# SokhengDin/DNN-MPPI-MPC

Hardware: NVIDIA B200
Metric: mppi_sample_steps_per_sec (higher is better)
Workload: dtype f32

## Files before the change

dnn-mppi-mpc_b200/csrc/mppi_api.cu:

```cuda
#include <cuda_runtime.h>
#include <dlfcn.h>
#include <nccl.h>

#include <algorithm>
#include <cmath>
#include <cstdio>
#include <cstdlib>
#include <cstring>
#include <string>
#include <vector>

#include "mppi_device.cuh"
#include "mppi_launch.h"
#include "mppi_mlp.h"

namespace {

struct NcclApi {
    void *lib = nullptr;
    ncclResult_t (*GetUniqueId)(ncclUniqueId *) = nullptr;
    ncclResult_t (*CommInitRank)(ncclComm_t *, int, ncclUniqueId, int) = nullptr;
    ncclResult_t (*AllGather)(const void *, void *, size_t, ncclDataType_t, ncclComm_t, cudaStream_t) = nullptr;
    ncclResult_t (*CommDestroy)(ncclComm_t) = nullptr;
    const char *(*GetErrorString)(ncclResult_t) = nullptr;
// ... 281 lines not shown
            h->grid_x_tpar = gt;
            gx = std::max(gx, gt);
        }
    }

    CKC(gmalloc(h, &h->d_U, sizeof(float) * R * T * 2));
    CKC(cudaMemset(h->d_U, 0, sizeof(float) * R * T * 2));
    CKC(gmalloc(h, &h->d_M, sizeof(float) * T * T));
    CKC(gmalloc(h, &h->d_S, sizeof(float) * (size_t)R * K));
    CKC(gmalloc(h, &h->d_NC, sizeof(int) * (size_t)K));
    const int gmax = (gx + MPPI_MERGE_GROUP_CTAS - 1) / MPPI_MERGE_GROUP_CTAS;
    CKC(gmalloc(h, &h->d_part, sizeof(float) * (size_t)R * (gx + gmax) * MPPI_NF(T)));
    CKC(gmalloc(h, &h->d_out, sizeof(float) * (size_t)R * MPPI_OUT_STRIDE));
    CKC(cudaMemset(h->d_out, 0, sizeof(float) * (size_t)R * MPPI_OUT_STRIDE));
    CKC(gmalloc(h, &h->d_idx, sizeof(int) * R));
    CKC(cudaMemset(h->d_idx, 0, sizeof(int) * R));
    CKC(gmalloc(h, &h->d_ticket, sizeof(unsigned) * (size_t)R * (1 + gmax)));
    CKC(cudaMemset(h->d_ticket, 0, sizeof(unsigned) * (size_t)R * (1 + gmax)));
    CKC(cudaHostAlloc(&h->h_out, sizeof(float) * MPPI_OUT_STRIDE, cudaHostAllocMapped));
    std::memset(h->h_out, 0, sizeof(float) * MPPI_OUT_STRIDE);
    CKC(cudaHostGetDevicePointer(&h->h_out_dev, h->h_out, 0));
    CKC(gmalloc(h, &h->d_first, sizeof(unsigned long long)));
    CKC(cudaHostAlloc(&h->h_first, sizeof(unsigned long long), cudaHostAllocDefault));
    h->idx_mirror = 0; h->idx_mirror_ok = true;
    for (auto &e : h->ev) CKC(cudaEventCreate(&e));
    std::vector<float> M;
    build_filter(T, c.filter_kind, M);
    CKC(cudaMemcpy(h->d_M, M.data(), sizeof(float) * T * T, cudaMemcpyHostToDevice));

    TickArgs &a = h->args;
    std::memset(&a, 0, sizeof(a));
    a.K = K; a.T = T; a.window = c.window; a.yaw_wrap = c.yaw_wrap; a.clamp_nominal = c.clamp_nominal;
    a.k_offset = c.k_offset;
    {
        const double thr = (1.0 - c.param_exploration) * (double)c.K_global;
        long long n = (long long)std::ceil(thr);
        n = std::max(0LL, std::min((long long)c.K_global, n));
        a.n_exploit = (int)n;
    }
    a.dt = (float)c.dt; a.dt_over_L = (float)(c.dt / c.wheel_base);
    a.umax0 = (float)c.u_max[0]; a.umax1 = (float)c.u_max[1];
    for (int i = 0; i < 4; ++i) { a.sw[i] = (float)c.stage_w[i]; a.tw[i] = (float)c.term_w[i]; }
    const double gamma = c.param_lambda * (1.0 - c.param_alpha);
    a.use_gamma = gamma != 0.0;
    a.gq[0] = (float)(gamma * c.sigma[3] / det); a.gq[1] = (float)(-gamma * c.sigma[1] / det);
    a.gq[2] = (float)(-gamma * c.sigma[2] / det); a.gq[3] = (float)(gamma * c.sigma[0] / det);
    const double l00 = std::sqrt(c.sigma[0]), l10 = c.sigma[2] / l00;
    a.chol[0] = (float)l00; a.chol[1] = (float)l10; a.chol[2] = (float)std::sqrt(c.sigma[3] - l10 * l10);
    a.inv_temp = (float)(1.0 / c.temperature);
    for (int i = 0; i < 4; ++i) a.goal[i] = (float)c.goal[i];
    a.ctrl_w[0] = (float)c.ctrl_w[0]; a.ctrl_w[1] = (float)c.ctrl_w[1];
    a.soft_w = (float)c.soft_obs_weight; a.soft_sd = (float)c.soft_obs_safety;
    refresh_obstacle_args(h, nullptr, 0);
    a.U = h->d_U; a.idx = h->d_idx; a.M = h->d_M; a.part = h->d_part; a.ticket = h->d_ticket;
    a.part2 = h->d_part + (size_t)R * gx * MPPI_NF(T); a.ticket2 = h->d_ticket + R; a.merge_gmax = gmax;
    a.out = h->d_out; a.out_host = h->h_out_dev;
    if (c.model == MPPI_MODEL_DIFFDRIVE_MLP) {
        h->mlp = mlp_create(K, T);
        if (!h->mlp) { mppi_destroy(h); return MPPI_E_CUDA; }
    }
#undef CKC
    *out = h;
    return MPPI_OK;
}

int mppi_destroy(mppi_handle_t h) {
// ... 755 lines not shown
```

dnn-mppi-mpc_b200/csrc/mppi_device.cuh:

```cuda
#pragma once
#include <cuda_runtime.h>
#include <stdint.h>
#include <math_constants.h>
#include "../../include/mppi_b200.h"

#ifndef MPPI_DEBUG_CHECKS
#define MPPI_DEBUG_CHECKS 0
#endif
#if MPPI_DEBUG_CHECKS
#include <assert.h>
#define MPPI_DCHECK(c) assert(c)
#else
#define MPPI_DCHECK(c) ((void)0)
#endif
#ifndef MPPI_BLOCK
#define MPPI_BLOCK 256
#endif
#define MPPI_WARPS (MPPI_BLOCK / 32)
#ifndef MPPI_SPT
#define MPPI_SPT 1
#endif
#define MPPI_CHUNK (MPPI_BLOCK * MPPI_SPT)
#ifndef MPPI_MIN_BLOCKS
#define MPPI_MIN_BLOCKS (MPPI_BLOCK >= 512 ? 1 : 768 / MPPI_BLOCK)
// ... 17 lines not shown
#define MPPI_XCHG_TOTAL (MPPI_XCHG_BARRIER + MPPI_MAX_PEERS)

enum : int {
    F_WRITE_S = 1,
    F_UPDATE = 2,
    F_FROM_S = 4,
    F_HOST_IDX = 8,
    F_TRIPLE_OUT = 16,
    F_KEEP_IDX = 32,
    F_IDX_ONLY = 64,
    F_P2P = 128,
    F_COST_SUM = 0x10000
};

struct TickArgs {
    int K, T, window, n_path, n_obs, yaw_wrap, use_gamma, clamp_nominal;
    int k_offset, n_exploit;
    float dt, dt_over_L, umax0, umax1;
    float sw[4], tw[4];
    float gq[4];
    float chol[3];
    float inv_temp;
    float obs_x[MPPI_MAX_OBSTACLES], obs_y[MPPI_MAX_OBSTACLES];
    float obs_r2[MPPI_MAX_OBSTACLES];
    float obs_far2[MPPI_MAX_OBSTACLES];
    float fp_hl, fp_hw;
    float goal[4];
    float ctrl_w[2];
    float soft_w, soft_sd;
    float obs_vx[MPPI_MAX_OBSTACLES], obs_vy[MPPI_MAX_OBSTACLES];
    float x0[4];
    uint32_t seed_lo, seed_hi, tick;
    int idx_host, flags;
    const float4 *path;
    const int *path_len;
    int path_stride;
    const float *x0_dev;
    float *U;
    int *idx;
    const float *M;
    const float *eps;
    float *S;
    int *NC;
    float *S_user;
    float *part;
    unsigned *ticket;
    float *part2;
    unsigned *ticket2;
    int merge_gmax;
    float *out;
    float *out_host;
    float *u0_out;
    float *triple_out;
    float *plant_state;
    float *plant_log;
    int plant_mode, plant_tick, plant_n;
    unsigned *loop_state;
    unsigned *loop_ticket;
    unsigned long long *peer_buf[MPPI_MAX_PEERS];
    int p2p_rank, p2p_world;
    unsigned p2p_seq;
    unsigned p2p_timeout_ms;
    unsigned long long *trace;
};

__device__ __forceinline__ void philox4x32_10(uint32_t &c0, uint32_t &c1, uint32_t &c2, uint32_t &c3,
// ... 324 lines not shown
#endif
    auto far = [&](int ch) {
        const float4 cb = sm.cb[ch];
        const float ex = x - cb.x, ey = y - cb.y, R = sbm + cb.z;
        return fmaf(ey, ey, ex * ex) > R * R * 1.0002f;
    };
#if MPPI_WP_CHUNK_ILP
    for (; c + 1 < nch; c += 2) {
        if (far(c) && far(c + 1)) continue;
        float m0, k0, m1, k1;
        chunk_argmin<16>(nwx4 + 4 * c, nwy4 + 4 * c, x, y, m0, k0);
        chunk_argmin<16>(nwx4 + 4 * c + 4, nwy4 + 4 * c + 4, x, y, m1, k1);
        const bool second = m1 < m0;
        const float m = second ? m1 : m0;
        const int j = second ? 16 * c + 16 + __float2int_rn(k1) : 16 * c + __float2int_rn(k0);
        if (m < bm) { bm = m; bj = j; sbm = sqrtf(m); }
    }
#endif
    for (; c < nch; ++c) {
        if (far(c)) continue;
        float m, key;
        chunk_argmin<16>(nwx4 + 4 * c, nwy4 + 4 * c, x, y, m, key);
        if (m < bm) { bm = m; bj = 16 * c + __float2int_rn(key); sbm = sqrtf(m); }
    }
    return bj;
}

__device__ __forceinline__ float4 window_ref(const TickSmem &sm, int j) {
    MPPI_DCHECK(j >= 0 && j < MPPI_MAX_WINDOW);
    const float2 yv = sm.wyv[j];
    return make_float4(-sm.wx[j], -sm.wy[j], yv.x, yv.y);
}

__device__ __forceinline__ void sincos_cw(float x, float &s, float &c) {
    const float t = fmaf(x, 0.636619772f, 12582912.f);
    const int q = __float_as_int(t);
    const float k = t - 12582912.f;
    float r = fmaf(k, -1.5707963705062866f, x);
    r = fmaf(k, 4.371138828673793e-08f, r);
    r = fmaf(k, 1.7151245100058819e-15f, r);
    const float r2 = r * r;
    float sp = fmaf(r2, -1.9515295891e-4f, 8.3321608736e-3f);
    sp = fmaf(sp, r2, -1.6666654611e-1f);
    sp = fmaf(sp * r2, r, r);
    float cp = fmaf(r2, 2.443315711809948e-5f, -1.388731625493765e-3f);
    cp = fmaf(cp, r2, 4.166664568298827e-2f);
    cp = fmaf(cp, r2, -0.5f);
    cp = fmaf(cp, r2, 1.0f);
    const float ss = (q & 1) ? cp : sp, cc = (q & 1) ? sp : cp;
    s = __int_as_float(__float_as_int(ss) ^ ((q << 30) & 0x80000000));
    c = __int_as_float(__float_as_int(cc) ^ (((q + 1) << 30) & 0x80000000));
}

__device__ __forceinline__ float wrap_2pi(float yaw) {
    const float b = 6.2831855f;
    const float y2 = yaw + b;
    const float q = floorf(y2 * 0.15915494f);
    float r = fmaf(-q, b, y2);
    if (r < 0.f) r += b;
    if (r >= b) r -= b;
    return r;
}

template <int MODEL, int COLL>
__device__ __forceinline__ bool collided(const TickArgs &a, float x, float y, float cs, float sn) {
    bool hit = false;
// ... 37 lines not shown
#define MPPI_WIN_GOAL (-1)
#define MPPI_WIN_TARGET (-2)

__device__ __forceinline__ float goal_cost(const TickArgs &a, const float z[4], const float w[4]) {
    const float dx = z[0] - a.goal[0], dy = z[1] - a.goal[1];
    const float d2 = fmaf(dy, dy, dx * dx);
    const float diff = atan2f(dy, dx) - z[2];
    const float k = rintf(diff * 0.15915494309189535f);
    float r = fmaf(k, -6.2831854820251465f, diff);
    r = fmaf(k, 1.7484555314695172e-07f, r);
    return w[0] * d2 + w[1] * r * r;
}

__device__ __forceinline__ float target_soft_cost(const TickArgs &a, const float z[4], float v0, float v1, int t,
                                                  const float w[4], bool full) {
    const float ex = z[0] - a.goal[0], ey = z[1] - a.goal[1], eth = z[2] - a.goal[2];
    float c = w[0] * ex * ex + w[1] * ey * ey + w[2] * eth * eth;
    if (full) {
        c += a.ctrl_w[0] * v0 * v0 + a.ctrl_w[1] * v1 * v1;
        const float tt = (float)t * a.dt;
        float soft = 0.f;
        for (int m = 0; m < a.n_obs; ++m) {
            const float dx = z[0] - fmaf(a.obs_vx[m], tt, a.obs_x[m]), dy = z[1] - fmaf(a.obs_vy[m], tt, a.obs_y[m]);
            const float d = sqrtf(fmaf(dy, dy, dx * dx));
            if (d < a.soft_sd) soft += expf(a.soft_sd - d);
        }
        c = fmaf(a.soft_w, soft, c);
    }
    return c;
}

template <int MODEL, int WIN>
__device__ __forceinline__ float eval_state_cost(const TickArgs &a, const TickSmem &sm, const float z[4], float v0, float v1,
                                                 int t, const float w[4], float4 &ref, float &yaw_eff) {
    if constexpr (WIN == MPPI_WIN_GOAL) {
        return goal_cost(a, z, w);
    } else if constexpr (WIN == MPPI_WIN_TARGET) {
        return target_soft_cost(a, z, v0, v1, t, w, true);
    } else {
        const int j = nearest_wp<WIN>(sm, z[0], z[1]);
        ref = window_ref(sm, j);
        yaw_eff = (MODEL == MPPI_MODEL_BICYCLE && a.yaw_wrap) ? wrap_2pi(z[2]) : z[2];
        return tracking_cost<MODEL>(ref, z, yaw_eff, w);
    }
}
template <int MODEL, int WIN>
__device__ __forceinline__ float eval_terminal_cost(const TickArgs &a, const float z[4], const float4 ref, float yaw_eff) {
    if constexpr (WIN == MPPI_WIN_GOAL) return goal_cost(a, z, a.tw);
    else if constexpr (WIN == MPPI_WIN_TARGET) return target_soft_cost(a, z, 0.f, 0.f, 0, a.tw, false);
    else return tracking_cost<MODEL>(ref, z, yaw_eff, a.tw);
}

template <int MODEL>
__device__ __forceinline__ void dyn_step(const TickArgs &a, float z[4], float v0, float v1, float cs, float sn) {
    if (MODEL == MPPI_MODEL_BICYCLE) {
        const float vel = z[3];
        z[0] += vel * cs * a.dt;
        z[1] += vel * sn * a.dt;
        z[2] += vel * a.dt_over_L * tanf(v0);
        z[3] += v1 * a.dt;
    } else {
        z[0] += v0 * cs * a.dt;
        z[1] += v0 * sn * a.dt;
        z[2] += v1 * a.dt;
    }
}

template <int MODEL>
__device__ __forceinline__ void dyn_step_tan(const TickArgs &a, float z[4], float v0, float v1, float cs, float sn, float tan_v0) {
    if (MODEL == MPPI_MODEL_BICYCLE) {
        const float vel = z[3];
        z[0] += vel * cs * a.dt;
        z[1] += vel * sn * a.dt;
        z[2] += vel * a.dt_over_L * tan_v0;
        z[3] += v1 * a.dt;
    } else {
        dyn_step<MODEL>(a, z, v0, v1, cs, sn);
    }
}

__device__ __forceinline__ float clampf(float v, float lim) { return fminf(fmaxf(v, -lim), lim); }

template <int MODEL, int COLL, bool SUM, bool INJ, int WIN, int SPT>
__device__ __forceinline__ void rollout_samples(const TickArgs &a, const TickSmem &sm, const uint32_t (&kg)[SPT], const int (&klocal)[SPT],
                                                uint32_t robot, const bool (&exploit)[SPT], float2 *stash, float (&smooth)[SPT], int (&ncoll)[SPT],
                                                uint32_t tick_add = 0u) {
    const int T = a.T;
    float z[SPT][4], cs[SPT], sn[SPT], acc[SPT], v0[SPT], v1[SPT], yaw_eff[SPT];
    int nc[SPT];
    float4 ref[SPT];
    bool hit[SPT];
    const float2 *eps_k[SPT];
#pragma unroll
    for (int s = 0; s < SPT; ++s) {
        z[s][0] = sm.x0[0]; z[s][1] = sm.x0[1]; z[s][2] = sm.x0[2]; z[s][3] = sm.x0[3];
        sincos_cw(z[s][2], sn[s], cs[s]);
        acc[s] = 0.f; nc[s] = 0; v0[s] = v1[s] = 0.f; yaw_eff[s] = 0.f; hit[s] = false;
        ref[s] = make_float4(0.f, 0.f, 0.f, 0.f);
        eps_k[s] = INJ ? reinterpret_cast<const float2 *>(a.eps) + (size_t)klocal[s] * T : nullptr;
    }

    auto fetch = [&](int s, int tp, float e[4]) {
        if (INJ) {
            e[0] = e[1] = e[2] = e[3] = 0.f;
            if (tp < T) { const float2 ea = eps_k[s][tp]; e[0] = ea.x; e[1] = ea.y; }
            if (tp + 1 < T) { const float2 eb = eps_k[s][tp + 1]; e[2] = eb.x; e[3] = eb.y; }
        } else {
            philox_eps_pair(a, kg[s], (uint32_t)(tp >> 1), robot, e, tick_add);
        }
    };
    auto step = [&](int s, int t, float e0, float e1) {
        MPPI_DCHECK(t >= 0 && t < T);
        if (stash) stash[t * MPPI_CHUNK + s * MPPI_BLOCK] = make_float2(e0, e1);
        const float2 u = sm.U[t];
        v0[s] = clampf(exploit[s] ? __fadd_rn(u.x, e0) : e0, a.umax0);
        v1[s] = clampf(exploit[s] ? __fadd_rn(u.y, e1) : e1, a.umax1);
        dyn_step<MODEL>(a, z[s], v0[s], v1[s], cs[s], sn[s]);
        sincos_cw(z[s][2], sn[s], cs[s]);
        if (SUM) {
            const float c = eval_state_cost<MODEL, WIN>(a, sm, z[s], v0[s], v1[s], t, a.sw, ref[s], yaw_eff[s]);
            const float2 q = sm.Q[t];
            acc[s] += c + (q.x * v0[s] + q.y * v1[s]);
            hit[s] = collided<MODEL, COLL>(a, z[s][0], z[s][1], cs[s], sn[s]);
            nc[s] += hit[s] ? 1 : 0;
        }
    };

    float e[SPT][4];
#pragma unroll
    for (int s = 0; s < SPT; ++s) fetch(s, 0, e[s]);
    const int n_fetch_pairs = WIN >= 0 ? (T - 1) >> 1 : T >> 1;
    int tp = 0;
    for (int i = 0; i < n_fetch_pairs; ++i, tp += 2) {
        float en[SPT][4];
#pragma unroll
        for (int s = 0; s < SPT; ++s) fetch(s, tp + 2, en[s]);
#pragma unroll
        for (int s = 0; s < SPT; ++s) step(s, tp, e[s][0], e[s][1]);
#pragma unroll
        for (int s = 0; s < SPT; ++s) step(s, tp + 1, e[s][2], e[s][3]);
#pragma unroll
        for (int s = 0; s < SPT; ++s) { e[s][0] = en[s][0]; e[s][1] = en[s][1]; e[s][2] = en[s][2]; e[s][3] = en[s][3]; }
    }
#pragma unroll
    for (int s = 0; s < SPT; ++s) {
        if (WIN >= 0) {
            step(s, tp, e[s][0], e[s][1]);
            if (!(T & 1)) step(s, tp + 1, e[s][2], e[s][3]);
        } else if (T & 1) {
            step(s, T - 1, e[s][0], e[s][1]);
        }
        if (SUM) {
            acc[s] += eval_terminal_cost<MODEL, WIN>(a, z[s], ref[s], yaw_eff[s]);
            nc[s] += hit[s] ? 1 : 0;
        } else {
            const float2 q = sm.Q[T - 1];
            acc[s] = eval_state_cost<MODEL, WIN>(a, sm, z[s], v0[s], v1[s], T - 1, a.sw, ref[s], yaw_eff[s]) + (q.x * v0[s] + q.y * v1[s]);
            acc[s] += eval_terminal_cost<MODEL, WIN>(a, z[s], ref[s], yaw_eff[s]);
            nc[s] = collided<MODEL, COLL>(a, z[s][0], z[s][1], cs[s], sn[s]) ? 2 : 0;
        }
        smooth[s] = acc[s];
        ncoll[s] = nc[s];
    }
}

#define MPPI_TPAR_SLOTS 64
#ifndef MPPI_TPAR_PROBE
#define MPPI_TPAR_PROBE 0
#endif
#if MPPI_TPAR_PROBE
#include <cstdio>
#endif
struct TparSmem {
    int prog[MPPI_TPAR_SLOTS / 32];
    int next;
};
template <int MODEL, int COLL, int WIN>
__device__ __forceinline__ void rollout_tpar(const TickArgs &a, const TickSmem &sm, TparSmem &ts, const int k_begin, const int n, const uint32_t robot,
                                             float2 *stash, float4 *zbuf, float &smooth, int &ncoll, const uint32_t tick_add) {
    const int T = a.T, tid = threadIdx.x;
    const uint32_t inv_n = n > 1 ? (uint32_t)((0x100000000ull + (uint32_t)n - 1u) / (uint32_t)n) : 0u;
    auto div_n = [&](int i) { return n > 1 ? (int)__umulhi((uint32_t)i, inv_n) : i; };
    if (tid < MPPI_TPAR_SLOTS / 32) ts.prog[tid] = 0;
    if (tid == 0) ts.next = 0;
    const uint32_t kg0 = (uint32_t)(a.k_offset + k_begin);
    MPPI_DCHECK(n >= 1 && n <= MPPI_TPAR_SLOTS && MPPI_TPAR_SLOTS <= MPPI_BLOCK);
#if MPPI_TPAR_PROBE
    long long pc[5];
#define MPPI_TPAR_STAMP(i) pc[i] = clock64()
#else
#define MPPI_TPAR_STAMP(i)
#endif
    MPPI_TPAR_STAMP(0);
    {
        const int npairs = (T + 1) >> 1, items = n * npairs;
        for (int i = tid; i < items; i += MPPI_BLOCK) {
            const int p = div_n(i), slot = i - p * n;
            MPPI_DCHECK(p == i / n && 2 * p < T && slot >= 0 && slot < n);
            float e[4];
            philox_eps_pair(a, kg0 + (uint32_t)slot, (uint32_t)p, robot, e, tick_add);
            stash[(2 * p) * MPPI_TPAR_SLOTS + slot] = make_float2(e[0], e[1]);
            if (2 * p + 1 < T) stash[(2 * p + 1) * MPPI_TPAR_SLOTS + slot] = make_float2(e[2], e[3]);
            if (MODEL == MPPI_MODEL_BICYCLE) {
                const bool exploit = (int)(kg0 + (uint32_t)slot) < a.n_exploit;
                const float ua = sm.U[2 * p].x, ub = (2 * p + 1 < T) ? sm.U[2 * p + 1].x : 0.f;
                zbuf[(2 * p) * MPPI_TPAR_SLOTS + slot].x = tanf(clampf(exploit ? __fadd_rn(ua, e[0]) : e[0], a.umax0));
                if (2 * p + 1 < T) zbuf[(2 * p + 1) * MPPI_TPAR_SLOTS + slot].x = tanf(clampf(exploit ? __fadd_rn(ub, e[2]) : e[2], a.umax0));
            }
        }
        const int idle = MPPI_TPAR_SLOTS - n;
        for (int i = tid; i < idle * T; i += MPPI_BLOCK) {
            const int t = i / idle, slot = n + (i - t * idle);
// ... 28 lines not shown
                asm volatile("st.release.cta.shared.u32 [%0], %1;" ::"r"((uint32_t)__cvta_generic_to_shared(&ts.prog[warp])), "r"(done) : "memory");
            }
        }
    }
    MPPI_TPAR_STAMP(2);
    {
        const int items = n * T;
        for (;;) {
            int base = 0;
            if (lane == 0) base = atomicAdd(&ts.next, 32);
            base = __shfl_sync(0xffffffffu, base, 0);
            if (base >= items) break;
            const int i = base + lane;
            if (i < items) {
                const int t = div_n(i), slot = i - t * n;
                MPPI_DCHECK(t == i / n && t < T && slot >= 0 && slot < n && (slot >> 5) < n_dw);
                {
                    const uint32_t flag = (uint32_t)__cvta_generic_to_shared(&ts.prog[slot >> 5]);
                    int done;
                    for (;;) {
                        asm volatile("ld.acquire.cta.shared.u32 %0, [%1];" : "=r"(done) : "r"(flag) : "memory");
                        if (done > t) break;
                        __nanosleep(40);
                    }
                }
                const float4 z4 = zbuf[t * MPPI_TPAR_SLOTS + slot];
                const float z[4] = {z4.x, z4.y, z4.z, z4.w};
                const bool exploit = (int)(kg0 + (uint32_t)slot) < a.n_exploit;
                const float2 e = stash[t * MPPI_TPAR_SLOTS + slot], u = sm.U[t];
                const float v0 = clampf(exploit ? __fadd_rn(u.x, e.x) : e.x, a.umax0);
                const float v1 = clampf(exploit ? __fadd_rn(u.y, e.y) : e.y, a.umax1);
                float4 ref = make_float4(0.f, 0.f, 0.f, 0.f);
                float yaw_eff = 0.f;
                const float c = eval_state_cost<MODEL, WIN>(a, sm, z, v0, v1, t, a.sw, ref, yaw_eff);
                const float2 q = sm.Q[t];
                const float cc = c + (q.x * v0 + q.y * v1);
                bool hit = false;
                if constexpr (COLL != MPPI_COLLISION_NONE) {
                    float cs, sn;
                    sincos_cw(z[2], sn, cs);
                    hit = collided<MODEL, COLL>(a, z[0], z[1], cs, sn);
                }
                const float term = (t == T - 1) ? eval_terminal_cost<MODEL, WIN>(a, z, ref, yaw_eff) : 0.f;
                zbuf[t * MPPI_TPAR_SLOTS + slot] = make_float4(cc, term, hit ? 1.f : 0.f, 0.f);
            }
        }
    }
    __syncthreads();
    MPPI_TPAR_STAMP(3);
    smooth = CUDART_INF_F; ncoll = INT_MAX;
    if (tid < n) {
        float acc = 0.f;
        int nc = 0;
        float4 r = make_float4(0.f, 0.f, 0.f, 0.f);
        for (int t = 0; t < T; ++t) {
            r = zbuf[t * MPPI_TPAR_SLOTS + tid];
            acc += r.x;
            nc += (r.z != 0.f) ? 1 : 0;
        }
        acc += r.y;
        nc += (r.z != 0.f) ? 1 : 0;
        smooth = acc; ncoll = nc;
    }
#if MPPI_TPAR_PROBE
    MPPI_TPAR_STAMP(4);
    if (tid == 0 && (blockIdx.x == 0 || blockIdx.x == 77) && a.tick == 25u)
        printf("tpar block %d n %d: N %lld D %lld C %lld S %lld cycles\n", (int)blockIdx.x, n, pc[1] - pc[0], pc[2] - pc[1], pc[3] - pc[2], pc[4] - pc[3]);
// ... 3 lines not shown
```

dnn-mppi-mpc_b200/csrc/mppi_kernels.cu:

```cuda
#include "mppi_device.cuh"
#include "mppi_launch.h"

#include <algorithm>

namespace {

__device__ __forceinline__ float warp_sum(float v) {
#pragma unroll
    for (int o = 16; o > 0; o >>= 1) v += __shfl_xor_sync(0xffffffffu, v, o);
    return v;
}

__device__ __forceinline__ void warp_lexmin(int &n, float &s) {
    const int nmin = __reduce_min_sync(0xffffffffu, n);
    float c = (n == nmin) ? s : CUDART_INF_F;
#pragma unroll
    for (int o = 16; o > 0; o >>= 1) c = fminf(c, __shfl_xor_sync(0xffffffffu, c, o));
    n = nmin; s = c;
}

__device__ __forceinline__ float rel_weight(int n, float s, int n0, float s0, float inv_temp) {
    const float d = (float)(n - n0) * MPPI_PENALTY + (s - s0);
    return __expf(-d * inv_temp);
}

struct MergeSmem {
    float red_s[MPPI_WARPS];
    int red_n[MPPI_WARPS];
    float col[4 + 2 * MPPI_MAX_T];
    float weps[2 * MPPI_MAX_T];
    float upre[2 * MPPI_MAX_T];
};

#ifndef MPPI_MERGE_TWO_LEVEL
#define MPPI_MERGE_TWO_LEVEL 1
#endif
#define MPPI_MERGE_TWO_LEVEL_MIN 64
#define MPPI_MERGE_TILE 1000
#define MPPI_MERGE_GROUPS 4
#define MPPI_MERGE_SCRATCH (MPPI_MERGE_TILE + MPPI_MERGE_GROUPS * MPPI_NF_MAX)
static_assert(4 * MPPI_BLOCK <= MPPI_MERGE_SCRATCH || MPPI_BLOCK > 256, "merge fast path: group sums must fit the scratch");
__device__ void merge_partials(const TickArgs &a, const float *parts, int P, MergeSmem &ms, float *sc, int stride = 0) {
    const int tid = threadIdx.x, lane = tid & 31, warp = tid >> 5;
    const int NF = MPPI_NF(a.T);
    if (stride == 0) stride = NF;
    int n = INT_MAX;
    float s = CUDART_INF_F;
    int my_n = INT_MAX;
    float my_s = CUDART_INF_F;
    for (int p = tid; p < P; p += MPPI_BLOCK) {
        const int pn = __float_as_int(__ldcg(parts + (size_t)p * stride));
        const float ps = __ldcg(parts + (size_t)p * stride + 1);
        if (p == tid) { my_n = pn; my_s = ps; }
        if (pn < n || (pn == n && ps < s)) { n = pn; s = ps; }
    }
    warp_lexmin(n, s);
    if (lane == 0) { ms.red_n[warp] = n; ms.red_s[warp] = s; }
    __syncthreads();
    n = ms.red_n[0]; s = ms.red_s[0];
#pragma unroll
    for (int w = 1; w < MPPI_WARPS; ++w) {
        const int wn = ms.red_n[w]; const float ws = ms.red_s[w];
        if (wn < n || (wn == n && ws < s)) { n = wn; s = ws; }
    }
    if ((NF & 3) == 0 && (stride & 3) == 0 && MPPI_BLOCK / (NF >> 2) >= 2 && P <= MPPI_MERGE_TILE) {
        const int NQ = NF >> 2, G4 = min(MPPI_BLOCK / NQ, 16);
        const int g4 = tid / NQ, cq = tid - g4 * NQ;
        __syncthreads();
        if (tid < P) sc[tid] = rel_weight(my_n, my_s, n, s, a.inv_temp);
        for (int p = tid + MPPI_BLOCK; p < P; p += MPPI_BLOCK) {
            const float *pp = parts + (size_t)p * stride;
            sc[p] = rel_weight(__float_as_int(__ldcg(pp)), __ldcg(pp + 1), n, s, a.inv_temp);
        }
// ... 161 lines not shown
            } else {
                const float steer = clampf(u0x, a.umax0), accel = clampf(u0y, a.umax1);
                px += pv * cs * a.dt; py += pv * sn * a.dt; pyaw += pv * a.dt_over_L * tanf(steer); pv += accel * a.dt;
            }
            ps[0] = px; ps[1] = py; ps[2] = pyaw; ps[3] = pv;
            float *lg = a.plant_log + 4 * ((size_t)(pt + 1) * R + robot);
            lg[0] = px; lg[1] = py; lg[2] = pyaw; lg[3] = pv;
            float *lu = a.plant_log + 4 * (size_t)(a.plant_n + 1) * R + 2 * ((size_t)pt * R + robot);
            lu[0] = u0x; lu[1] = u0y;
        }
        if (!(a.flags & F_KEEP_IDX)) a.idx[robot] = idx_new;
    }
}

struct RunSmem {
    int n;
    float s;
    float eta, e2;
    float N[2 * MPPI_MAX_T];
    float w[MPPI_CHUNK];
    float warp_eta[MPPI_WARPS], warp_e2[MPPI_WARPS];
    float red_s[MPPI_WARPS];
    int red_n[MPPI_WARPS];
    unsigned long long key[MPPI_WARPS];
    unsigned ticket;
};

extern __shared__ __align__(16) unsigned char mppi_dyn_smem[];

template <int MODEL, int COLL, bool SUM, bool INJ, int WIN, int STASH>
__device__ __forceinline__ void tick_body(const TickArgs &a, const uint32_t tick_add) {
    __shared__ TickSmem sm;
    __shared__ RunSmem run;
    __shared__ MergeSmem ms;
    float2 *stash = reinterpret_cast<float2 *>(mppi_dyn_smem);
    float (*warpN)[2 * MPPI_MAX_T] = reinterpret_cast<float (*)[2 * MPPI_MAX_T]>(mppi_dyn_smem);
    const int tid = threadIdx.x, lane = tid & 31, warp = tid >> 5;
    const int robot = blockIdx.y, b = blockIdx.x, B = gridDim.x;
    const int T = a.T, K = a.K;

    if (a.trace && tid == 0 && robot == 0) { unsigned long long t; asm volatile("mov.u64 %0, %%globaltimer;" : "=l"(t)); a.trace[2 * b] = t; }
    if (tid < 4) sm.x0[tid] = a.x0_dev ? a.x0_dev[robot * 4 + tid] : a.x0[tid];
    __syncthreads();
    const float4 *rpath = a.path_len ? a.path + (size_t)robot * a.path_stride : a.path;
    const int n_path = a.path_len ? a.path_len[robot] : a.n_path;
    int s_new;
    if (WIN < 0) {
        s_new = 0;
    } else if (a.flags & F_HOST_IDX) {
        s_new = a.idx_host;
    } else {
        const int s_old = max(0, min(a.idx[robot], n_path - 1));
        unsigned long long key = ~0ull;
        MPPI_DCHECK(n_path >= 1 && s_old >= 0 && s_old < n_path && a.window <= MPPI_MAX_WINDOW);
        for (int j = tid; j < a.window && s_old + j < n_path; j += MPPI_BLOCK) {
            const float4 p = rpath[s_old + j];
            const float dx = sm.x0[0] - p.x, dy = sm.x0[1] - p.y;
            const unsigned long long kj = ((unsigned long long)__float_as_uint(dx * dx + dy * dy) << 32) | (unsigned)j;
            key = kj < key ? kj : key;
        }
#pragma unroll
        for (int o = 16; o > 0; o >>= 1) {
            const unsigned long long other = __shfl_xor_sync(0xffffffffu, key, o);
            key = other < key ? other : key;
        }
        if (lane == 0) run.key[warp] = key;
        __syncthreads();
        key = run.key[0];
#pragma unroll
        for (int w = 1; w < MPPI_WARPS; ++w) key = run.key[w] < key ? run.key[w] : key;
        s_new = s_old + (int)(key & 0xffffffffu);
    }
    {
        int nw = n_path - s_new; nw = nw < a.window ? nw : a.window;
        MPPI_DCHECK(WIN < 0 || (s_new >= 0 && s_new < n_path && nw >= 1));
        const int fill = (WIN < 0) ? 0 : (WIN == 20) ? 20 : MPPI_WP_FULL ? ((nw + 63) & ~63) : ((nw + 15) & ~15);
        for (int j = tid; j < fill; j += MPPI_BLOCK) {
            if (j < nw) {
                const float4 p = rpath[s_new + j];
                sm.wx[j] = -p.x; sm.wy[j] = -p.y; sm.wyv[j] = make_float2(p.z, p.w);
            } else {
                sm.wx[j] = -MPPI_SENTINEL; sm.wy[j] = -MPPI_SENTINEL; sm.wyv[j] = make_float2(0.f, 0.f);
            }
        }
        if (tid == 0) { sm.win_start = s_new; sm.n_win16 = fill >> 4; }
#if MPPI_WIN20_EXPANDED
        if (WIN == 20) { __syncthreads(); fill_window_expanded(sm, nw, tid, MPPI_BLOCK); }
#endif
        if (WIN == 0) {
            __syncthreads();
            for (int c = tid; c < (fill >> 4); c += MPPI_BLOCK) sm.cb[c] = chunk_bound(sm.wx, sm.wy, 16 * c, min(16, nw - 16 * c));
        }
        const float *Ur = a.U + (size_t)robot * T * 2;
        for (int t = tid; t < T; t += MPPI_BLOCK) {
            const float u0 = Ur[2 * t], u1 = Ur[2 * t + 1];
            sm.U[t] = make_float2(u0, u1);
            sm.Q[t] = make_float2(u0 * a.gq[0] + u1 * a.gq[2], u0 * a.gq[1] + u1 * a.gq[3]);
        }
        if (tid == 0) { run.n = INT_MAX; run.s = CUDART_INF_F; run.eta = 0.f; run.e2 = 0.f; }
        for (int c = tid; c < 2 * T; c += MPPI_BLOCK) run.N[c] = 0.f;
    }
    __syncthreads();

    constexpr int SPT = MPPI_SPT;
    const int k_begin = (int)((long long)K * b / B);
    const int k_end = (a.flags & F_IDX_ONLY) ? k_begin : (int)((long long)K * (b + 1) / B);
    MPPI_DCHECK(k_begin >= 0 && k_end <= K && (!STASH || (size_t)T * MPPI_CHUNK * sizeof(float2) <= 232448));
    float *Srow = a.S ? a.S + (size_t)robot * K : nullptr;
    static_assert(STASH != 2 || (SPT == 1 && SUM && !INJ), "time-parallel rollout: one sample per thread, sum mode, Philox noise");
    constexpr int CHUNK_STRIDE = STASH == 2 ? MPPI_TPAR_SLOTS : MPPI_CHUNK;
    for (int base = k_begin; base < k_end; base += CHUNK_STRIDE) {
        int k[SPT], ksafe[SPT], ncoll[SPT];
        bool active[SPT], exploit[SPT];
        uint32_t kg[SPT];
        float smooth[SPT];
#pragma unroll
        for (int s = 0; s < SPT; ++s) {
            k[s] = base + tid + s * MPPI_BLOCK;
            active[s] = k[s] < k_end && (STASH != 2 || tid < MPPI_TPAR_SLOTS);
            ksafe[s] = active[s] ? k[s] : k_begin;
            kg[s] = (uint32_t)(a.k_offset + ksafe[s]);
            exploit[s] = (int)kg[s] < a.n_exploit;
            smooth[s] = CUDART_INF_F; ncoll[s] = INT_MAX;
        }
        if constexpr (STASH == 2) {
            MPPI_DCHECK(!(a.flags & F_FROM_S) && (size_t)T * MPPI_TPAR_SLOTS * (sizeof(float2) + sizeof(float4)) <= 232448);
            float4 *zbuf = reinterpret_cast<float4 *>(mppi_dyn_smem + sizeof(float2) * (size_t)T * MPPI_TPAR_SLOTS);
            __shared__ TparSmem tps;
            rollout_tpar<MODEL, COLL, WIN>(a, sm, tps, base, min(k_end - base, MPPI_TPAR_SLOTS), (uint32_t)robot, stash, zbuf,
                                           smooth[0], ncoll[0], tick_add);
            if (active[0] && (a.flags & F_WRITE_S)) Srow[k[0]] = smooth[0] + MPPI_PENALTY * (float)ncoll[0];
        } else if (active[0]) {
            if (a.flags & F_FROM_S) {
#pragma unroll
                for (int s = 0; s < SPT; ++s)
                    if (active[s]) { smooth[s] = Srow[k[s]]; ncoll[s] = a.NC ? a.NC[k[s]] : 0; }
            } else {
                rollout_samples<MODEL, COLL, SUM, INJ, WIN, SPT>(a, sm, kg, ksafe, (uint32_t)robot, exploit,
                                                                 STASH ? stash + tid : nullptr, smooth, ncoll, tick_add);
#pragma unroll
                for (int s = 0; s < SPT; ++s) {
                    if (active[s] && (a.flags & F_WRITE_S)) Srow[k[s]] = smooth[s] + MPPI_PENALTY * (float)ncoll[s];
                    if (!active[s]) { smooth[s] = CUDART_INF_F; ncoll[s] = INT_MAX; }
                }
            }
        }
        if (!(a.flags & F_UPDATE)) continue;
        if (STASH == 1 && !active[0]) {
            for (int t = 0; t < T; ++t)
#pragma unroll
                for (int s = 0; s < SPT; ++s) stash[t * MPPI_CHUNK + s * MPPI_BLOCK + tid] = make_float2(0.f, 0.f);
        }

        int cn = ncoll[0]; float cs_ = smooth[0];
#pragma unroll
        for (int s = 1; s < SPT; ++s)
            if (ncoll[s] < cn || (ncoll[s] == cn && smooth[s] < cs_)) { cn = ncoll[s]; cs_ = smooth[s]; }
        warp_lexmin(cn, cs_);
        if (lane == 0) { run.red_n[warp] = cn; run.red_s[warp] = cs_; }
        __syncthreads();
        int mn = run.n; float mss = run.s;
#pragma unroll
        for (int w = 0; w < MPPI_WARPS; ++w) {
            const int wn = run.red_n[w]; const float ws = run.red_s[w];
            if (wn < mn || (wn == mn && ws < mss)) { mn = wn; mss = ws; }
        }
        const float rescale = (run.n == INT_MAX) ? 0.f : rel_weight(run.n, run.s, mn, mss, a.inv_temp);
        float w[SPT], wsum = 0.f, w2sum = 0.f;
#pragma unroll
        for (int s = 0; s < SPT; ++s) {
            w[s] = active[s] ? rel_weight(ncoll[s], smooth[s], mn, mss, a.inv_temp) : 0.f;
            wsum += w[s]; w2sum = fmaf(w[s], w[s], w2sum);
// ... 406 lines not shown
    } else {
        if (inj) { if (win20) MPPI_PICK(false, true, 20, false); else MPPI_PICK(false, true, 0, false); }
        if (stash) { if (win20) MPPI_PICK(false, false, 20, true); else MPPI_PICK(false, false, 0, true); }
        if (win20) MPPI_PICK(false, false, 20, false); else MPPI_PICK(false, false, 0, false);
    }
#undef MPPI_PICK
}

template <typename F>
static cudaError_t with_tick_kernel(int model, int coll, int cost_kind, bool sum, bool inj, bool win20, int stash, F &&f) {
    if (cost_kind == MPPI_COSTKIND_GOAL) {
        if (model != MPPI_MODEL_DIFFDRIVE) return cudaErrorInvalidValue;
        if (coll == MPPI_COLLISION_NONE) return with_tick_kernel_nopath<MPPI_COLLISION_NONE, MPPI_WIN_GOAL>(sum, inj, stash, f);
        if (coll == MPPI_COLLISION_CIRCLE) return with_tick_kernel_nopath<MPPI_COLLISION_CIRCLE, MPPI_WIN_GOAL>(sum, inj, stash, f);
        return cudaErrorInvalidValue;
    }
    if (cost_kind == MPPI_COSTKIND_TARGET_SOFT) {
        if (model != MPPI_MODEL_DIFFDRIVE || coll != MPPI_COLLISION_NONE) return cudaErrorInvalidValue;
        return with_tick_kernel_nopath<MPPI_COLLISION_NONE, MPPI_WIN_TARGET>(sum, inj, stash, f);
    }
    if (model == MPPI_MODEL_DIFFDRIVE) {
        if (coll == MPPI_COLLISION_NONE) return with_tick_kernel_mc<MPPI_MODEL_DIFFDRIVE, MPPI_COLLISION_NONE>(sum, inj, win20, stash, f);
        if (coll == MPPI_COLLISION_CIRCLE) return with_tick_kernel_mc<MPPI_MODEL_DIFFDRIVE, MPPI_COLLISION_CIRCLE>(sum, inj, win20, stash, f);
    } else if (model == MPPI_MODEL_BICYCLE) {
        if (coll == MPPI_COLLISION_NONE) return with_tick_kernel_mc<MPPI_MODEL_BICYCLE, MPPI_COLLISION_NONE>(sum, inj, win20, stash, f);
        if (coll == MPPI_COLLISION_CIRCLE) return with_tick_kernel_mc<MPPI_MODEL_BICYCLE, MPPI_COLLISION_CIRCLE>(sum, inj, win20, stash, f);
        if (coll == MPPI_COLLISION_FOOTPRINT) return with_tick_kernel_mc<MPPI_MODEL_BICYCLE, MPPI_COLLISION_FOOTPRINT>(sum, inj, win20, stash, f);
    }
    return cudaErrorInvalidValue;
}

size_t mppi_tick_dyn_smem(int T, int stash) {
    const size_t small = std::max(sizeof(float) * MPPI_WARPS * 2 * MPPI_MAX_T, sizeof(float) * MPPI_MAX_PEERS * MPPI_NF_MAX);
    if (stash == 2) return std::max((sizeof(float2) + sizeof(float4)) * MPPI_TPAR_SLOTS * (size_t)T, small);
    return stash ? std::max(sizeof(float2) * (size_t)T * MPPI_CHUNK, small) : small;
}

cudaError_t mppi_launch_tick(const TickArgs &a, int model, int coll, int cost_kind, bool sum, bool inj, int stash, dim3 grid, cudaStream_t st) {
    const size_t dyn = mppi_tick_dyn_smem(a.T, stash);
    return with_tick_kernel(model, coll, cost_kind, sum, inj, a.window == 20, stash, [&](auto kern) {
        if (dyn > 32 * 1024) {
            static thread_local const void *done_kern[64];
            static thread_local size_t done_dyn[64];
            static thread_local int done_dev[64], n_done = 0;
            int dev = 0;
            cudaGetDevice(&dev);
            bool found = false;
            for (int i = 0; i < n_done; ++i)
                if (done_kern[i] == (const void *)kern && done_dev[i] == dev && done_dyn[i] >= dyn) { found = true; break; }
            if (!found) {
                cudaError_t e = cudaFuncSetAttribute(kern, cudaFuncAttributeMaxDynamicSharedMemorySize, (int)dyn);
                if (e != cudaSuccess) return e;
                if (n_done < 64) { done_kern[n_done] = (const void *)kern; done_dyn[n_done] = dyn; done_dev[n_done] = dev; ++n_done; }
            }
        }
        kern<<<grid, MPPI_BLOCK, dyn, st>>>(a);
        return cudaGetLastError();
    });
}

int mppi_tick_occupancy(int model, int coll, int cost_kind, bool sum, bool inj, int window, int T, int stash) {
    int nb = 0;
    const size_t dyn = mppi_tick_dyn_smem(T, stash);
    cudaError_t e = with_tick_kernel(model, coll, cost_kind, sum, inj, window == 20, stash, [&](auto kern) {
        if (dyn > 32 * 1024) {
            cudaError_t e2 = cudaFuncSetAttribute(kern, cudaFuncAttributeMaxDynamicSharedMemorySize, (int)dyn);
            if (e2 != cudaSuccess) return e2;
        }
// ... 23 lines not shown
                               unsigned long long *first_change, cudaStream_t st) {
    if (model == MPPI_MODEL_DIFFDRIVE) {
        if (coll == MPPI_COLLISION_NONE) return launch_strict_mc<MPPI_MODEL_DIFFDRIVE, MPPI_COLLISION_NONE>(a, sum, inj, bp_n, bp_s, nbp, k_first, check_from, first_change, st);
        if (coll == MPPI_COLLISION_CIRCLE) return launch_strict_mc<MPPI_MODEL_DIFFDRIVE, MPPI_COLLISION_CIRCLE>(a, sum, inj, bp_n, bp_s, nbp, k_first, check_from, first_change, st);
    } else if (model == MPPI_MODEL_BICYCLE) {
        if (coll == MPPI_COLLISION_NONE) return launch_strict_mc<MPPI_MODEL_BICYCLE, MPPI_COLLISION_NONE>(a, sum, inj, bp_n, bp_s, nbp, k_first, check_from, first_change, st);
        if (coll == MPPI_COLLISION_FOOTPRINT) return launch_strict_mc<MPPI_MODEL_BICYCLE, MPPI_COLLISION_FOOTPRINT>(a, sum, inj, bp_n, bp_s, nbp, k_first, check_from, first_change, st);
    }
    return cudaErrorInvalidValue;
}

cudaError_t mppi_launch_p2p_barrier(const TickArgs &a, unsigned long long count, cudaStream_t st) {
    mppi_p2p_barrier_kernel<<<1, 32, 0, st>>>(a, count);
    return cudaGetLastError();
}

cudaError_t mppi_launch_merge(const TickArgs &a, const float *triples, int G, cudaStream_t st) {
    mppi_merge_kernel<<<1, MPPI_BLOCK, 0, st>>>(a, triples, G);
    return cudaGetLastError();
}

cudaError_t mppi_launch_traj(const TickArgs &a, int model, const float *rec, float *d_opt, float *d_samp,
                             const int *d_sel, int n_sel, int shift, cudaStream_t st) {
    const int n = (d_sel ? n_sel : a.K) + 1;
    if (model == MPPI_MODEL_BICYCLE) mppi_traj_kernel<MPPI_MODEL_BICYCLE><<<(n + 127) / 128, 128, 0, st>>>(a, rec, d_opt, d_samp, d_sel, n_sel, shift);
    else mppi_traj_kernel<MPPI_MODEL_DIFFDRIVE><<<(n + 127) / 128, 128, 0, st>>>(a, rec, d_opt, d_samp, d_sel, n_sel, shift);
    return cudaGetLastError();
}

cudaError_t mppi_launch_noise(const TickArgs &a, float *d_out, int robot, cudaStream_t st) {
    mppi_noise_kernel<<<(a.K + 255) / 256, 256, 0, st>>>(a, d_out, robot);
    return cudaGetLastError();
}
```

Measured before the change: 125.6 billion.

## Add grid-accelerated nearest-waypoint lookup for 20-point tracking window

Builds a 16x16 grid over the expanded window's point space, where each cell stores a conservative 4-row candidate range of waypoints that could be nearest. Rollouts then evaluate only 4 candidates instead of all 20, and fall back to the full search when any lane in the warp is out of bounds or lands in an unresolved cell. The merge shared state moves into dynamic shared memory at a fixed offset to make room for the grid. This adds per-block build cost and more shared memory, and is gated on a minimum per-block workload and an env toggle.

Measured after the change: 131.0 billion (median of 6 runs). +4.3%, better.

```diff
diff --git a/dnn-mppi-mpc_b200/csrc/mppi_api.cu b/dnn-mppi-mpc_b200/csrc/mppi_api.cu
--- a/dnn-mppi-mpc_b200/csrc/mppi_api.cu
+++ b/dnn-mppi-mpc_b200/csrc/mppi_api.cu
@@ -337,6 +337,8 @@
     std::memset(&a, 0, sizeof(a));
     a.K = K; a.T = T; a.window = c.window; a.yaw_wrap = c.yaw_wrap; a.clamp_nominal = c.clamp_nominal;
     a.k_offset = c.k_offset;
+    a.wp_fast = 1;
+    if (const char *env = std::getenv("MPPI_WP_FAST")) a.wp_fast = std::atoi(env) != 0;
     {
         const double thr = (1.0 - c.param_exploration) * (double)c.K_global;
         long long n = (long long)std::ceil(thr);
diff --git a/dnn-mppi-mpc_b200/csrc/mppi_device.cuh b/dnn-mppi-mpc_b200/csrc/mppi_device.cuh
--- a/dnn-mppi-mpc_b200/csrc/mppi_device.cuh
+++ b/dnn-mppi-mpc_b200/csrc/mppi_device.cuh
@@ -73,6 +73,7 @@
     float x0[4];
     uint32_t seed_lo, seed_hi, tick;
     int idx_host, flags;
+    int wp_fast;
     const float4 *path;
     const int *path_len;
     int path_stride;
@@ -463,6 +464,128 @@
     return make_float4(-sm.wx[j], -sm.wy[j], yv.x, yv.y);
 }
 
+#ifndef MPPI_WP_FAST
+#define MPPI_WP_FAST 1
+#endif
+#ifndef MPPI_WP_FAST_PROBE
+#define MPPI_WP_FAST_PROBE 0
+#endif
+#define MPPI_WP_GRID 16
+#define MPPI_WP_ROWS 4
+#define MPPI_WP_MARK 0xff
+#ifndef MPPI_WP_FAST_MIN_WORK
+#define MPPI_WP_FAST_MIN_WORK 65536
+#endif
+struct WpFastSmem {
+    float4 row[20];
+    float gx0, gy0, gihx, gihy;
+    unsigned char lo[MPPI_WP_GRID * MPPI_WP_GRID];
+};
+
+#if MPPI_WP_FAST_PROBE
+static __device__ unsigned long long mppi_wp_probe_count[5];
+#endif
+
+__device__ __forceinline__ void wp_fast_build(const TickSmem &sm, WpFastSmem &wf, int nw, int tid, int nthreads) {
+    float xmin = CUDART_INF_F, xmax = -CUDART_INF_F, ymin = CUDART_INF_F, ymax = -CUDART_INF_F;
+    for (int j = 0; j < nw && j < 20; ++j) {
+        const float px = -2.f * sm.ex[j], py = -2.f * sm.ey[j];
+        xmin = fminf(xmin, px); xmax = fmaxf(xmax, px); ymin = fminf(ymin, py); ymax = fmaxf(ymax, py);
+    }
+    const float ext = fmaxf(fmaxf(xmax - xmin, ymax - ymin), 1e-3f);
+    const float gx0 = xmin - 0.5f * ext, gy0 = ymin - 0.5f * ext;
+    const float hx = (xmax - xmin + ext) * (1.f / MPPI_WP_GRID), hy = (ymax - ymin + ext) * (1.f / MPPI_WP_GRID);
+    if (tid == 0) { wf.gx0 = gx0; wf.gy0 = gy0; wf.gihx = 1.f / hx; wf.gihy = 1.f / hy; }
+    for (int j = tid; j < 20; j += nthreads) wf.row[j] = make_float4(sm.ex[j], sm.ey[j], sm.ec[j], (float)j);
+    for (int cell = tid; cell < MPPI_WP_GRID * MPPI_WP_GRID; cell += nthreads) {
+        const int ix = cell % MPPI_WP_GRID, iy = cell / MPPI_WP_GRID;
+        const float xa = gx0 + ((float)ix - 0.015625f) * hx, xb = gx0 + ((float)ix + 1.015625f) * hx;
+        const float ya = gy0 + ((float)iy - 0.015625f) * hy, yb = gy0 + ((float)iy + 1.015625f) * hy;
+        const float cx[4] = {xa, xb, xa, xb}, cy[4] = {ya, ya, yb, yb};
+        int ic[4] = {0, 0, 0, 0};
+        float best[4] = {CUDART_INF_F, CUDART_INF_F, CUDART_INF_F, CUDART_INF_F};
+        for (int j = 0; j < 20; ++j) {
+            const float ex = sm.ex[j], ey = sm.ey[j], ec = sm.ec[j];
+#pragma unroll
+            for (int c = 0; c < 4; ++c) {
+                const float d = fmaf(ey, cy[c], fmaf(ex, cx[c], ec));
+                if (d < best[c]) { best[c] = d; ic[c] = j; }
+            }
+        }
+        const unsigned icp = (unsigned)ic[0] | (unsigned)ic[1] << 5 | (unsigned)ic[2] << 10 | (unsigned)ic[3] << 15;
+        auto dominated = [&](int j) {
+            const float exj = sm.ex[j], eyj = sm.ey[j], ecj = sm.ec[j];
+            bool any = false;
+#pragma unroll
+            for (int k = 0; k < 4; ++k) {
+                const int i = (icp >> (5 * k)) & 31;
+                MPPI_DCHECK(i < 20);
+                const float exi = sm.ex[i], eyi = sm.ey[i], eci = sm.ec[i];
+                bool all = true;
+#pragma unroll
+                for (int c = 0; c < 4; ++c) {
+                    const float D = (eci - ecj) + (exi - exj) * cx[c] + (eyi - eyj) * cy[c];
+                    const float S = fabsf(eci) + fabsf(ecj) + (fabsf(exi) + fabsf(exj)) * fabsf(cx[c]) + (fabsf(eyi) + fabsf(eyj)) * fabsf(cy[c]);
+                    all = all && (fmaf(0x1p-18f, S, D) + 0x1p-88f < 0.f);
+                }
+                any = any || all;
+            }
+            return any;
+        };
+        const int imin = min(min(ic[0], ic[1]), min(ic[2], ic[3])), imax = max(max(ic[0], ic[1]), max(ic[2], ic[3]));
+        int lo = MPPI_WP_MARK;
+        if (imax - imin < MPPI_WP_ROWS) {
+            int l = imin, h = imax;
+            for (int j = 0; j < imin; ++j) if (!dominated(j)) { l = j; break; }
+            if (imax - l < MPPI_WP_ROWS)
+                for (int j = 19; j > imax; --j) if (!dominated(j)) { h = j; break; }
+            if (h - l < MPPI_WP_ROWS) lo = min(l, 20 - MPPI_WP_ROWS);
+        }
+        wf.lo[cell] = (unsigned char)lo;
+    }
+}
+
+__device__ __forceinline__ int nearest_wp20_fast(const TickSmem &sm, const WpFastSmem &wf, float x, float y) {
+    const float ax = fmaf(-2.f, x, sm.c2x), ay = fmaf(-2.f, y, sm.c2y);
+    const float fx = (ax - wf.gx0) * wf.gihx, fy = (ay - wf.gy0) * wf.gihy;
+    const bool inb = fx >= 0.f && fx < (float)MPPI_WP_GRID && fy >= 0.f && fy < (float)MPPI_WP_GRID;
+    const int cx = min(max((int)fx, 0), MPPI_WP_GRID - 1), cy = min(max((int)fy, 0), MPPI_WP_GRID - 1);
+    MPPI_DCHECK(cx >= 0 && cx < MPPI_WP_GRID && cy >= 0 && cy < MPPI_WP_GRID);
+    const int lo = wf.lo[cy * MPPI_WP_GRID + cx];
+    const bool fast = inb && lo != MPPI_WP_MARK;
+    auto rows = [&]() {
+        const int l = min(lo, 20 - MPPI_WP_ROWS);
+        MPPI_DCHECK(l >= 0 && l + MPPI_WP_ROWS <= 20);
+        float d[MPPI_WP_ROWS], k[MPPI_WP_ROWS];
+        float4 r[MPPI_WP_ROWS];
+#pragma unroll
+        for (int q = 0; q < MPPI_WP_ROWS; ++q) {
+            r[q] = wf.row[l + q];
+            d[q] = __fmaf_rn(r[q].y, ay, __fmaf_rn(r[q].x, ax, r[q].z));
+        }
+        const float m = fminf(fminf(d[0], d[1]), fminf(d[2], d[3]));
+#pragma unroll
+        for (int q = 0; q < MPPI_WP_ROWS; ++q) k[q] = __fmaf_rn(__fadd_rn(d[q], -m), 1.2676506e30f, r[q].w);
+        return __float2int_rn(fminf(fminf(k[0], k[1]), fminf(k[2], k[3])));
+    };
+#if MPPI_WP_FAST_PROBE
+    {
+        const unsigned am = __activemask();
+        const bool fin = isfinite(ax) && isfinite(ay);
+        const int full = nearest_wp<20>(sm, x, y);
+        const unsigned bad = __ballot_sync(am, fast && rows() != full);
+        const int reason = __all_sync(am, fast) ? 0 : !__all_sync(am, fin) ? 1 : !__all_sync(am, inb) ? 2 : 3;
+        if ((threadIdx.x & 31) == __ffs(am) - 1) {
+            atomicAdd(&mppi_wp_probe_count[reason], 1ull);
+            if (bad) atomicAdd(&mppi_wp_probe_count[4], (unsigned long long)__popc(bad));
+        }
+        return full;
+    }
+#endif
+    if (__all_sync(__activemask(), fast)) return rows();
+    return nearest_wp<20>(sm, x, y);
+}
+
 __device__ __forceinline__ void sincos_cw(float x, float &s, float &c) {
     const float t = fmaf(x, 0.636619772f, 12582912.f);
     const int q = __float_as_int(t);
@@ -566,13 +689,18 @@
 
 template <int MODEL, int WIN>
 __device__ __forceinline__ float eval_state_cost(const TickArgs &a, const TickSmem &sm, const float z[4], float v0, float v1,
-                                                 int t, const float w[4], float4 &ref, float &yaw_eff) {
+                                                 int t, const float w[4], float4 &ref, float &yaw_eff,
+                                                 const WpFastSmem &wf, bool wf_on) {
     if constexpr (WIN == MPPI_WIN_GOAL) {
         return goal_cost(a, z, w);
     } else if constexpr (WIN == MPPI_WIN_TARGET) {
         return target_soft_cost(a, z, v0, v1, t, w, true);
     } else {
+#if MPPI_WP_FAST
+        const int j = (WIN == 20 && wf_on) ? nearest_wp20_fast(sm, wf, z[0], z[1]) : nearest_wp<WIN>(sm, z[0], z[1]);
+#else
         const int j = nearest_wp<WIN>(sm, z[0], z[1]);
+#endif
         ref = window_ref(sm, j);
         yaw_eff = (MODEL == MPPI_MODEL_BICYCLE && a.yaw_wrap) ? wrap_2pi(z[2]) : z[2];
         return tracking_cost<MODEL>(ref, z, yaw_eff, w);
@@ -618,7 +746,7 @@
 template <int MODEL, int COLL, bool SUM, bool INJ, int WIN, int SPT>
 __device__ __forceinline__ void rollout_samples(const TickArgs &a, const TickSmem &sm, const uint32_t (&kg)[SPT], const int (&klocal)[SPT],
                                                 uint32_t robot, const bool (&exploit)[SPT], float2 *stash, float (&smooth)[SPT], int (&ncoll)[SPT],
-                                                uint32_t tick_add = 0u) {
+                                                const WpFastSmem &wf, bool wf_on, uint32_t tick_add = 0u) {
     const int T = a.T;
     float z[SPT][4], cs[SPT], sn[SPT], acc[SPT], v0[SPT], v1[SPT], yaw_eff[SPT];
     int nc[SPT];
@@ -652,7 +780,7 @@
         dyn_step<MODEL>(a, z[s], v0[s], v1[s], cs[s], sn[s]);
         sincos_cw(z[s][2], sn[s], cs[s]);
         if (SUM) {
-            const float c = eval_state_cost<MODEL, WIN>(a, sm, z[s], v0[s], v1[s], t, a.sw, ref[s], yaw_eff[s]);
+            const float c = eval_state_cost<MODEL, WIN>(a, sm, z[s], v0[s], v1[s], t, a.sw, ref[s], yaw_eff[s], wf, wf_on);
             const float2 q = sm.Q[t];
             acc[s] += c + (q.x * v0[s] + q.y * v1[s]);
             hit[s] = collided<MODEL, COLL>(a, z[s][0], z[s][1], cs[s], sn[s]);
@@ -689,7 +817,7 @@
             nc[s] += hit[s] ? 1 : 0;
         } else {
             const float2 q = sm.Q[T - 1];
-            acc[s] = eval_state_cost<MODEL, WIN>(a, sm, z[s], v0[s], v1[s], T - 1, a.sw, ref[s], yaw_eff[s]) + (q.x * v0[s] + q.y * v1[s]);
+            acc[s] = eval_state_cost<MODEL, WIN>(a, sm, z[s], v0[s], v1[s], T - 1, a.sw, ref[s], yaw_eff[s], wf, wf_on) + (q.x * v0[s] + q.y * v1[s]);
             acc[s] += eval_terminal_cost<MODEL, WIN>(a, z[s], ref[s], yaw_eff[s]);
             nc[s] = collided<MODEL, COLL>(a, z[s][0], z[s][1], cs[s], sn[s]) ? 2 : 0;
         }
@@ -711,7 +839,8 @@
 };
 template <int MODEL, int COLL, int WIN>
 __device__ __forceinline__ void rollout_tpar(const TickArgs &a, const TickSmem &sm, TparSmem &ts, const int k_begin, const int n, const uint32_t robot,
-                                             float2 *stash, float4 *zbuf, float &smooth, int &ncoll, const uint32_t tick_add) {
+                                             float2 *stash, float4 *zbuf, float &smooth, int &ncoll, const WpFastSmem &wf, bool wf_on,
+                                             const uint32_t tick_add) {
     const int T = a.T, tid = threadIdx.x;
     const uint32_t inv_n = n > 1 ? (uint32_t)((0x100000000ull + (uint32_t)n - 1u) / (uint32_t)n) : 0u;
     auto div_n = [&](int i) { return n > 1 ? (int)__umulhi((uint32_t)i, inv_n) : i; };
@@ -806,7 +935,7 @@
                 const float v1 = clampf(exploit ? __fadd_rn(u.y, e.y) : e.y, a.umax1);
                 float4 ref = make_float4(0.f, 0.f, 0.f, 0.f);
                 float yaw_eff = 0.f;
-                const float c = eval_state_cost<MODEL, WIN>(a, sm, z, v0, v1, t, a.sw, ref, yaw_eff);
+                const float c = eval_state_cost<MODEL, WIN>(a, sm, z, v0, v1, t, a.sw, ref, yaw_eff, wf, wf_on);
                 const float2 q = sm.Q[t];
                 const float cc = c + (q.x * v0 + q.y * v1);
                 bool hit = false;
diff --git a/dnn-mppi-mpc_b200/csrc/mppi_kernels.cu b/dnn-mppi-mpc_b200/csrc/mppi_kernels.cu
--- a/dnn-mppi-mpc_b200/csrc/mppi_kernels.cu
+++ b/dnn-mppi-mpc_b200/csrc/mppi_kernels.cu
@@ -39,6 +39,9 @@
 #define MPPI_MERGE_TILE 1000
 #define MPPI_MERGE_GROUPS 4
 #define MPPI_MERGE_SCRATCH (MPPI_MERGE_TILE + MPPI_MERGE_GROUPS * MPPI_NF_MAX)
+#define MPPI_MERGE_SMEM_OFF 8448
+static_assert(sizeof(float) * MPPI_MERGE_SCRATCH <= MPPI_MERGE_SMEM_OFF && sizeof(float) * MPPI_MAX_PEERS * MPPI_NF_MAX <= MPPI_MERGE_SMEM_OFF &&
+              MPPI_MERGE_SMEM_OFF % 16 == 0, "merge state overlaps the merge scratch");
 static_assert(4 * MPPI_BLOCK <= MPPI_MERGE_SCRATCH || MPPI_BLOCK > 256, "merge fast path: group sums must fit the scratch");
 __device__ void merge_partials(const TickArgs &a, const float *parts, int P, MergeSmem &ms, float *sc, int stride = 0) {
     const int tid = threadIdx.x, lane = tid & 31, warp = tid >> 5;
@@ -266,7 +269,8 @@
 __device__ __forceinline__ void tick_body(const TickArgs &a, const uint32_t tick_add) {
     __shared__ TickSmem sm;
     __shared__ RunSmem run;
-    __shared__ MergeSmem ms;
+    __shared__ WpFastSmem wf;
+    MergeSmem &ms = *reinterpret_cast<MergeSmem *>(mppi_dyn_smem + MPPI_MERGE_SMEM_OFF);
     float2 *stash = reinterpret_cast<float2 *>(mppi_dyn_smem);
     float (*warpN)[2 * MPPI_MAX_T] = reinterpret_cast<float (*)[2 * MPPI_MAX_T]>(mppi_dyn_smem);
     const int tid = threadIdx.x, lane = tid & 31, warp = tid >> 5;
@@ -277,6 +281,8 @@
     if (tid < 4) sm.x0[tid] = a.x0_dev ? a.x0_dev[robot * 4 + tid] : a.x0[tid];
     __syncthreads();
     const float4 *rpath = a.path_len ? a.path + (size_t)robot * a.path_stride : a.path;
+    const bool wf_on = MPPI_WP_FAST && MPPI_WIN20_EXPANDED && WIN == 20 && a.wp_fast &&
+                       ((long long)K * (b + 1) / B - (long long)K * b / B) * T >= MPPI_WP_FAST_MIN_WORK && !(a.flags & (F_IDX_ONLY | F_FROM_S));
     const int n_path = a.path_len ? a.path_len[robot] : a.n_path;
     int s_new;
     if (WIN < 0) {
@@ -321,6 +327,9 @@
 #if MPPI_WIN20_EXPANDED
         if (WIN == 20) { __syncthreads(); fill_window_expanded(sm, nw, tid, MPPI_BLOCK); }
 #endif
+#if MPPI_WP_FAST && MPPI_WIN20_EXPANDED
+        if (WIN == 20 && wf_on) { __syncthreads(); wp_fast_build(sm, wf, nw, tid, MPPI_BLOCK); }
+#endif
         if (WIN == 0) {
             __syncthreads();
             for (int c = tid; c < (fill >> 4); c += MPPI_BLOCK) sm.cb[c] = chunk_bound(sm.wx, sm.wy, 16 * c, min(16, nw - 16 * c));
@@ -362,7 +371,7 @@
             float4 *zbuf = reinterpret_cast<float4 *>(mppi_dyn_smem + sizeof(float2) * (size_t)T * MPPI_TPAR_SLOTS);
             __shared__ TparSmem tps;
             rollout_tpar<MODEL, COLL, WIN>(a, sm, tps, base, min(k_end - base, MPPI_TPAR_SLOTS), (uint32_t)robot, stash, zbuf,
-                                           smooth[0], ncoll[0], tick_add);
+                                           smooth[0], ncoll[0], wf, wf_on, tick_add);
             if (active[0] && (a.flags & F_WRITE_S)) Srow[k[0]] = smooth[0] + MPPI_PENALTY * (float)ncoll[0];
         } else if (active[0]) {
             if (a.flags & F_FROM_S) {
@@ -371,7 +380,7 @@
                     if (active[s]) { smooth[s] = Srow[k[s]]; ncoll[s] = a.NC ? a.NC[k[s]] : 0; }
             } else {
                 rollout_samples<MODEL, COLL, SUM, INJ, WIN, SPT>(a, sm, kg, ksafe, (uint32_t)robot, exploit,
-                                                                 STASH ? stash + tid : nullptr, smooth, ncoll, tick_add);
+                                                                 STASH ? stash + tid : nullptr, smooth, ncoll, wf, wf_on, tick_add);
 #pragma unroll
                 for (int s = 0; s < SPT; ++s) {
                     if (active[s] && (a.flags & F_WRITE_S)) Srow[k[s]] = smooth[s] + MPPI_PENALTY * (float)ncoll[s];
@@ -844,8 +853,9 @@
 
 size_t mppi_tick_dyn_smem(int T, int stash) {
     const size_t small = std::max(sizeof(float) * MPPI_WARPS * 2 * MPPI_MAX_T, sizeof(float) * MPPI_MAX_PEERS * MPPI_NF_MAX);
-    if (stash == 2) return std::max((sizeof(float2) + sizeof(float4)) * MPPI_TPAR_SLOTS * (size_t)T, small);
-    return stash ? std::max(sizeof(float2) * (size_t)T * MPPI_CHUNK, small) : small;
+    const size_t merge = MPPI_MERGE_SMEM_OFF + sizeof(MergeSmem);
+    if (stash == 2) return std::max((sizeof(float2) + sizeof(float4)) * MPPI_TPAR_SLOTS * (size_t)T, std::max(small, merge));
+    return std::max(stash ? sizeof(float2) * (size_t)T * MPPI_CHUNK : small, std::max(small, merge));
 }
 
 cudaError_t mppi_launch_tick(const TickArgs &a, int model, int coll, int cost_kind, bool sum, bool inj, int stash, dim3 grid, cudaStream_t st) {
@@ -935,3 +945,15 @@
     mppi_noise_kernel<<<(a.K + 255) / 256, 256, 0, st>>>(a, d_out, robot);
     return cudaGetLastError();
 }
+
+#if MPPI_WP_FAST_PROBE
+extern "C" int mppi_wp_probe_read(unsigned long long *out, int reset) {
+    if (cudaDeviceSynchronize() != cudaSuccess) return 1;
+    if (cudaMemcpyFromSymbol(out, mppi_wp_probe_count, sizeof(mppi_wp_probe_count)) != cudaSuccess) return 1;
+    if (reset) {
+        const unsigned long long zero[5] = {0, 0, 0, 0, 0};
+        if (cudaMemcpyToSymbol(mppi_wp_probe_count, zero, sizeof(zero)) != cudaSuccess) return 1;
+    }
+    return 0;
+}
+#endif
```
